# luo-yining/CFDBench

Measured on NVIDIA H100. Metric: fno_rollout_steps_per_sec, higher is better.
Workload: dtype bf16

## Files before the change

### cfdbench_b200/csrc/fno_block_fused.cu

```cuda
#include "fno_common.cuh"
#include "tc_common.cuh"
#include "tc_tma.cuh"
#include <math.h>
#include <string.h>

namespace fno {

constexpr int kFzRows = 16;
constexpr int kFzChunks = kH / kFzRows;
constexpr int kFzWgRows = kFzRows / 2;
constexpr int kFzThreads = 9 * 32;
constexpr int kFzProdWarp = 8;
constexpr int kZK = 2 * kM2;
constexpr int kImgK = 2 * kKX;
constexpr size_t kYmImgBytes = 147456;
constexpr uint32_t kFzStage = 4 * 6144;
constexpr int kFzFFloats = 2 * (2 * kFzRows) * kImgK;
constexpr int kFzEFloats = 2 * kW * kZK;
constexpr uint32_t kFzZtFloats = kC * kZK;
constexpr uint32_t kLboF = (2 * kFzRows / 8) * 128;
constexpr uint32_t kLboO = (kC / 8) * 128;
constexpr uint32_t kFzBoxW = kW, kFzBoxH = 1, kFzBoxC = kC;
constexpr uint32_t kFzRowBytes = kFzBoxW * kFzBoxH * kFzBoxC * 2;
constexpr int kFzXSlots = 4;
constexpr uint32_t kFzW0Bytes = kC * kC * 2;

__host__ __device__ constexpr int fz_x_slot(int n) { return n % kFzXSlots; }
__host__ __device__ constexpr uint32_t fz_x_parity(int n) { return static_cast<uint32_t>(n / kFzXSlots) & 1u; }

struct FzSmem {
  alignas(1024) unsigned char x[2][kFzXSlots][kFzRowBytes];
  alignas(1024) unsigned char st[2][2][kFzRowBytes];
  alignas(128) unsigned char y[2][kFzStage];
  alignas(128) float zt[kFzRows][2][kFzZtFloats];
  alignas(128) float f_hi[kFzFFloats / 2];
  alignas(128) float f_lo[kFzFFloats / 2];
  alignas(128) unsigned char w0[3][kFzW0Bytes];
  alignas(16) float bias[kC];
  alignas(8) uint64_t y_full[2], y_free[2];
  alignas(8) uint64_t x_full[2][kFzXSlots];
};
static_assert(sizeof(FzSmem) <= 232448, "block_fused_kernel: shared memory over the per-block opt-in limit");

__device__ __forceinline__ uint32_t sw128_bf16_offset(int line, int e) {
  return static_cast<uint32_t>(line * 128 + ((((e >> 3) ^ line) & 7) << 4) + (e & 7) * 2);
}

__global__ void __launch_bounds__(kFzThreads, 1)
    block_fused_kernel(const __grid_constant__ CUtensorMap x_map, const __grid_constant__ CUtensorMap out_map,
                       const unsigned char* __restrict__ img, const float* __restrict__ w0t,
                       const float* __restrict__ bias, const float* __restrict__ etab, const float* __restrict__ ftab,
                       int batch) {
  extern __shared__ __align__(1024) unsigned char smem_raw[];
  FzSmem& sm = *reinterpret_cast<FzSmem*>(smem_raw);
  if ((smem_u32(smem_raw) & 1023u) != 0) __trap();
  const int tid = threadIdx.x, lane = tid & 31, warp = tc::warp_index_uniform();
  const int chunk = blockIdx.x % kFzChunks, b0 = blockIdx.x / kFzChunks, bstride = gridDim.x / kFzChunks;
  const int n_units = b0 < batch ? (batch - b0 + bstride - 1) / bstride : 0;

  if (tid == 0) {
    for (int i = 0; i < 2; ++i) {
      mbar_init(&sm.y_full[i], 1);
      mbar_init(&sm.y_free[i], 4);
      for (int s = 0; s < kFzXSlots; ++s) mbar_init(&sm.x_full[i][s], 1);
    }
    fence_mbar_init();
  }
  for (int e = tid; e < kFzFFloats / 2; e += kFzThreads) {
    sm.f_hi[e] = __ldg(ftab + chunk * kFzFFloats + e);
    sm.f_lo[e] = __ldg(ftab + chunk * kFzFFloats + kFzFFloats / 2 + e);
  }
  for (int e = tid; e < kC * kC; e += kFzThreads) {
    const int i = e / kC, o = e % kC;
    const float w = w0t[e];
    const __nv_bfloat16 t1 = __float2bfloat16_rn(w);
    const float r1 = w - __bfloat162float(t1);
    const __nv_bfloat16 t2 = __float2bfloat16_rn(r1);
    const __nv_bfloat16 t3 = __float2bfloat16_rn(r1 - __bfloat162float(t2));
    const uint32_t off = static_cast<uint32_t>(((i >> 3) * (kC / 8) + (o >> 3)) * 128 + (o & 7) * 16 + (i & 7) * 2);
    *reinterpret_cast<__nv_bfloat16*>(sm.w0[0] + off) = t1;
    *reinterpret_cast<__nv_bfloat16*>(sm.w0[1] + off) = t2;
    *reinterpret_cast<__nv_bfloat16*>(sm.w0[2] + off) = t3;
  }
  if (tid < kC) sm.bias[tid] = bias != nullptr ? bias[tid] : 0.f;
  tc::fence_proxy_async_smem();
  __syncthreads();
  pdl_wait();
  pdl_launch_dependents();

  if (warp == kFzProdWarp) {
    if (lane < 2) {
      const int s = lane;
      for (int u = 0; u < n_units; ++u) {
        const unsigned char* src = img + static_cast<size_t>(b0 + u * bstride) * kYmImgBytes;
        for (int pi = 0; pi < 3; ++pi) {
          const int p = s + 2 * pi, f = 3 * u + pi;
          if (f >= 1) mbar_wait(&sm.y_free[s], (f - 1) & 1);
          mbar_expect_tx(&sm.y_full[s], kFzStage);
          bulk_g2s(sm.y[s], src + p * (kFzStage / 2), kFzStage / 2, &sm.y_full[s]);
          bulk_g2s(sm.y[s] + kFzStage / 2, src + kYmImgBytes / 2 + p * (kFzStage / 2), kFzStage / 2, &sm.y_full[s]);
        }
      }
    }
    return;
  }

  const int g = warp >> 2, wq = warp & 3, q = lane & 3, t = tid & 127;
  const int m0 = 16 * wq + (lane >> 2);
  const int n_fills = kFzWgRows * n_units;
  auto x_fill = [&](int n) {
    const int u = n / kFzWgRows, r = n % kFzWgRows, s = fz_x_slot(n);
    mbar_expect_tx(&sm.x_full[g][s], kFzRowBytes);
    tma_load_3d(sm.x[g][s], &x_map, 0, kFzRows * chunk + g + 2 * r, (b0 + u * bstride) * kC, &sm.x_full[g][s]);
  };
  if (t == 0)
    for (int n = 0; n < kFzXSlots && n < n_fills; ++n) x_fill(n);
  const uint32_t w0_s = tc::smem_addr(sm.w0[0]);
  uint32_t e_frag[2][kZK / 8][4];
#pragma unroll
  for (int hl = 0; hl < 2; ++hl)
#pragma unroll
    for (int ks = 0; ks < kZK / 8; ++ks)
#pragma unroll
      for (int j = 0; j < 4; ++j) {
        const uint32_t off = tc::kmajor_offset(m0 + 8 * (j & 1), 8 * ks + q + 4 * (j >> 1), kW) / 4;
        e_frag[hl][ks][j] = __float_as_uint(__ldg(etab + hl * (kFzEFloats / 2) + off));
      }

  for (int u = 0; u < n_units; ++u) {
    const int b = b0 + u * bstride;
    for (int pi = 0; pi < 3; ++pi) {
      const int p = g + 2 * pi, f = 3 * u + pi;
      mbar_wait(&sm.y_full[g], f & 1);
      uint32_t a_hi[6][4], a_lo[6][4];
#pragma unroll
      for (int ks = 0; ks < kImgK / 8; ++ks)
#pragma unroll
        for (int r = 0; r < 4; ++r) {
          const int m = m0 + 8 * (r & 1), kk = 8 * ks + q + 4 * (r >> 1), o = m & 31;
          const uint32_t off = (m >> 5) * 6144 + kk * 128 + (((o >> 3) ^ (kk & 3)) << 5) + (o & 7) * 4;
          a_hi[ks][r] = *reinterpret_cast<const uint32_t*>(sm.y[g] + off);
          a_lo[ks][r] = *reinterpret_cast<const uint32_t*>(sm.y[g] + kFzStage / 2 + off);
        }
      float acc[16];
      tc::wg_fence();
#pragma unroll
      for (int pass = 0; pass < 3; ++pass) {
        const uint32_t fb = tc::smem_addr(pass == 2 ? sm.f_lo : sm.f_hi);
#pragma unroll
        for (int ks = 0; ks < kImgK / 8; ++ks)
          tc::wg_tf32_rs_n32(acc, pass == 1 ? a_lo[ks] : a_hi[ks], tc::make_smem_desc(fb + ks * 2 * kLboF, kLboF, 128),
                             (pass | ks) ? 1u : 0u);
      }
      tc::wg_commit();
      __syncwarp();
      if (lane == 0) mbar_arrive(&sm.y_free[g]);
      tc::wg_wait<0>();
      tc::wg_fence_acc(acc);
      if (pi == 0) tc::named_barrier(1, 256);
#pragma unroll
      for (int hh = 0; hh < 2; ++hh) {
        const int m = m0 + 8 * hh, ky = 2 * p + (m >> 5), o = m & 31;
#pragma unroll
        for (int i = 0; i < 4; ++i)
#pragma unroll
          for (int e = 0; e < 2; ++e) {
            float v = acc[4 * i + 2 * hh + e];
            if (ky == 0 && e == 1) v = sm.bias[o];
            float hi, lo;
            tc::split_tf32(v, hi, lo);
            const uint32_t off = tc::kmajor_offset(o, 2 * ky + e, kC) / 4;
            sm.zt[4 * i + q][0][off] = hi;
            sm.zt[4 * i + q][1][off] = lo;
          }
      }
    }
    tc::fence_proxy_async_smem();
    tc::named_barrier(1, 256);

    float acc[2][16];
    uint32_t x_frag[2][kC / 16][4];
#pragma unroll
    for (int r = 0; r <= kFzWgRows; ++r) {
      if (r < kFzWgRows) {
        const int n = kFzWgRows * u + r, hl = g + 2 * r;
        mbar_wait(&sm.x_full[g][fz_x_slot(n)], fz_x_parity(n));
        const uint32_t a_x = tc::smem_addr(sm.x[g][fz_x_slot(n)]);
#pragma unroll
        for (int ks = 0; ks < kC / 16; ++ks)
          tc::ldmatrix_x4_trans(x_frag[r & 1][ks], a_x + sw128_bf16_offset(16 * ks + 8 * (lane >> 4) + (lane & 7),
                                                                             16 * wq + 8 * ((lane >> 3) & 1)));
        tc::wg_fence();
        const uint32_t b_z[3] = {tc::smem_addr(sm.zt[hl][0]), tc::smem_addr(sm.zt[hl][0]), tc::smem_addr(sm.zt[hl][1])};
#pragma unroll
        for (int pass = 0; pass < 3; ++pass)
#pragma unroll
          for (int ks = 0; ks < kZK / 8; ++ks)
            tc::wg_tf32_rs_n32(acc[r & 1], e_frag[pass == 1][ks],
                               tc::make_smem_desc(b_z[pass] + ks * 2 * kLboO, kLboO, 128), (pass | ks) ? 1u : 0u);
        tc::wg_fence();
#pragma unroll
        for (int term = 0; term < 3; ++term)
#pragma unroll
          for (int ks = 0; ks < kC / 16; ++ks)
            tc::wg_bf16_rs_n32(acc[r & 1], x_frag[r & 1][ks],
                               tc::make_smem_desc(w0_s + term * kFzW0Bytes + ks * 2 * kLboO, kLboO, 128), 1u);
        tc::wg_commit();
      }
      if (r == 0) continue;
      const int rr = r - 1, h = kFzRows * chunk + g + 2 * rr;
      float* d = acc[rr & 1];
      if (r < kFzWgRows) {
        tc::wg_wait<1>();
      } else {
        tc::wg_wait<0>();
      }
      tc::wg_fence_acc(acc[rr & 1]);
      unsigned char* stile = sm.st[g][rr & 1];
#pragma unroll
      for (int i2 = 0; i2 < 2; ++i2) {
        uint32_t v[4];
#pragma unroll
        for (int j = 0; j < 4; ++j) {
          const int i = 2 * i2 + (j >> 1), hh = j & 1;
          const float2 y = gelu_erf2(make_float2(d[4 * i + 2 * hh], d[4 * i + 2 * hh + 1]));
          const __nv_bfloat162 p = __floats2bfloat162_rn(y.x, y.y);
          v[j] = *reinterpret_cast<const uint32_t*>(&p);
        }
        tc::stmatrix_x4_trans(tc::smem_addr(stile) + sw128_bf16_offset(16 * i2 + 8 * (lane >> 4) + (lane & 7),
                                                                       16 * wq + 8 * ((lane >> 3) & 1)),
                              v);
      }
      tc::fence_proxy_async_smem();
      if (t == 0) bulk_wait_group_read<0>();
      tc::named_barrier(2 + g, 128);
      if (t == 0) {
        tma_store_3d(&out_map, stile, 0, h, b * kC);
        bulk_commit_group();
        const int nf = kFzWgRows * u + rr + kFzXSlots;
        if (nf < n_fills) x_fill(nf);
      }
    }
  }
  if (t == 0) bulk_wait_group<0>();
}

void c2r_operand_table(float* host, double s0, double s1);

static float fz_round_tf32_host(double v) {
  float f = static_cast<float>(v);
  uint32_t u;
  memcpy(&u, &f, 4);
  u = (u + 0x1000u) & 0xffffe000u;
  memcpy(&f, &u, 4);
  return f;
}

struct FzTables {
  float* etab = nullptr;
  float* ftab = nullptr;
  int n_sm = 0;
  bool configured = false;
};
static FzTables g_fz[64];

static cudaError_t fz_ensure(int dev, cudaStream_t stream) {
  FzTables& t = g_fz[dev];
  if (t.configured) return cudaSuccess;
  const double two_pi = 6.283185307179586476925286766559;
  static float h_e[kFzEFloats];
  static float h_f[kFzChunks * kFzFFloats];
  c2r_operand_table(h_e, 1.0 / kHW, 2.0 / kHW);
  for (int c = 0; c < kFzChunks; ++c)
    for (int n = 0; n < 2 * kFzRows; ++n) {
      const int h = kFzRows * c + (n >> 1), ri = n & 1;
      for (int k = 0; k < kImgK; ++k) {
        const int rip = k & 1, kxi = 2 * ((k % 24) >> 1) + k / 24, kx = kxi < kM1 ? kxi : kxi + (kH - kKX);
        const double ang = two_pi * ((kx * h) % 64) / 64.0;
        const double val = (ri == rip) ? cos(ang) : (ri == 0 ? -sin(ang) : sin(ang));
        const float hi = fz_round_tf32_host(val);
        const uint32_t off = tc::kmajor_offset(n, k, 2 * kFzRows) / 4;
        h_f[c * kFzFFloats + off] = hi;
        h_f[c * kFzFFloats + kFzFFloats / 2 + off] = fz_round_tf32_host(val - static_cast<double>(hi));
      }
    }
  cudaError_t e = cudaMalloc(&t.etab, sizeof(h_e));
  if (e != cudaSuccess) return e;
  e = cudaMalloc(&t.ftab, sizeof(h_f));
  if (e != cudaSuccess) return e;
  e = cudaMemcpyAsync(t.etab, h_e, sizeof(h_e), cudaMemcpyHostToDevice, stream);
  if (e != cudaSuccess) return e;
  e = cudaMemcpyAsync(t.ftab, h_f, sizeof(h_f), cudaMemcpyHostToDevice, stream);
  if (e != cudaSuccess) return e;
  e = cudaStreamSynchronize(stream);
  if (e != cudaSuccess) return e;
  e = cudaFuncSetAttribute(block_fused_kernel, cudaFuncAttributeMaxDynamicSharedMemorySize, (int)sizeof(FzSmem));
  if (e != cudaSuccess) return e;
  e = cudaDeviceGetAttribute(&t.n_sm, cudaDevAttrMultiProcessorCount, dev);
  if (e != cudaSuccess) return e;
  t.configured = true;
  return cudaSuccess;
}

void block_fused_release(int dev) {
  if (dev < 0 || dev >= 64) return;
  FzTables& t = g_fz[dev];
  if (t.etab) cudaFree(t.etab);
  if (t.ftab) cudaFree(t.ftab);
  t = FzTables();
}

cudaError_t launch_block_fused(const void* ym_img, const void* x, const float* w0t, const float* bias, void* out, int batch,
                               cudaStream_t stream) {
  int dev = 0;
  cudaError_t e = cudaGetDevice(&dev);
  if (e != cudaSuccess) return e;
  if (dev < 0 || dev >= 64) return cudaErrorInvalidDevice;
  e = fz_ensure(dev, stream);
  if (e != cudaSuccess) return e;
  if ((reinterpret_cast<uintptr_t>(x) & 15) || (reinterpret_cast<uintptr_t>(ym_img) & 15) ||
      (reinterpret_cast<uintptr_t>(out) & 15))
    return cudaErrorMisalignedAddress;
  CUtensorMap x_map, out_map;
  const uint64_t planes = static_cast<uint64_t>(batch) * kC;
  e = make_tma_map_3d(&x_map, CU_TENSOR_MAP_DATA_TYPE_BFLOAT16, 2, x, kW, kH, planes, kFzBoxW, kFzBoxH, kFzBoxC);
  if (e != cudaSuccess) return e;
  e = make_tma_map_3d(&out_map, CU_TENSOR_MAP_DATA_TYPE_BFLOAT16, 2, out, kW, kH, planes, kFzBoxW, kFzBoxH, kFzBoxC);
  if (e != cudaSuccess) return e;
  const int slots_max = g_fz[dev].n_sm / kFzChunks;
  const int slots = batch < slots_max ? batch : slots_max;
  return launch_chained(block_fused_kernel, dim3(kFzChunks * slots), dim3(kFzThreads), sizeof(FzSmem), stream, x_map,
                        out_map, static_cast<const unsigned char*>(ym_img), w0t, bias,
                        static_cast<const float*>(g_fz[dev].etab), static_cast<const float*>(g_fz[dev].ftab), batch);
}

}
```

Baseline: 1327.

## Drop producer warp, prefetch spectral image into registers during pointwise stage

Removes the dedicated TMA producer warp and has each warpgroup's thread 0 issue its own bulk copies of the spectral image. The image fragments for the next unit are loaded into registers while the pointwise/GEMM row loop of the current unit runs, and the three inverse-x MMA groups are issued back to back with staggered waits so their stores overlap the next MMA. The zt stores now use float4 vectors over a reorganised staging layout. The cost is much higher register pressure from holding three A-fragment sets, plus a single-slot y buffer whose reuse is now ordered by named barriers.

```diff
diff --git a/cfdbench_b200/csrc/fno_block_fused.cu b/cfdbench_b200/csrc/fno_block_fused.cu
--- a/cfdbench_b200/csrc/fno_block_fused.cu
+++ b/cfdbench_b200/csrc/fno_block_fused.cu
@@ -9,12 +9,12 @@
 constexpr int kFzRows = 16;
 constexpr int kFzChunks = kH / kFzRows;
 constexpr int kFzWgRows = kFzRows / 2;
-constexpr int kFzThreads = 9 * 32;
-constexpr int kFzProdWarp = 8;
+constexpr int kFzThreads = 8 * 32;
 constexpr int kZK = 2 * kM2;
 constexpr int kImgK = 2 * kKX;
 constexpr size_t kYmImgBytes = 147456;
-constexpr uint32_t kFzStage = 4 * 6144;
+constexpr uint32_t kImgKyBytes = kImgK * kC * 4;
+constexpr uint32_t kFzStage = 4 * kImgKyBytes;
 constexpr int kFzFFloats = 2 * (2 * kFzRows) * kImgK;
 constexpr int kFzEFloats = 2 * kW * kZK;
 constexpr uint32_t kFzZtFloats = kC * kZK;
@@ -37,7 +37,7 @@
   alignas(128) float f_lo[kFzFFloats / 2];
   alignas(128) unsigned char w0[3][kFzW0Bytes];
   alignas(16) float bias[kC];
-  alignas(8) uint64_t y_full[2], y_free[2];
+  alignas(8) uint64_t y_full[2];
   alignas(8) uint64_t x_full[2][kFzXSlots];
 };
 static_assert(sizeof(FzSmem) <= 232448, "block_fused_kernel: shared memory over the per-block opt-in limit");
@@ -61,7 +61,6 @@
   if (tid == 0) {
     for (int i = 0; i < 2; ++i) {
       mbar_init(&sm.y_full[i], 1);
-      mbar_init(&sm.y_free[i], 4);
       for (int s = 0; s < kFzXSlots; ++s) mbar_init(&sm.x_full[i][s], 1);
     }
     fence_mbar_init();
@@ -88,23 +87,6 @@
   pdl_wait();
   pdl_launch_dependents();
 
-  if (warp == kFzProdWarp) {
-    if (lane < 2) {
-      const int s = lane;
-      for (int u = 0; u < n_units; ++u) {
-        const unsigned char* src = img + static_cast<size_t>(b0 + u * bstride) * kYmImgBytes;
-        for (int pi = 0; pi < 3; ++pi) {
-          const int p = s + 2 * pi, f = 3 * u + pi;
-          if (f >= 1) mbar_wait(&sm.y_free[s], (f - 1) & 1);
-          mbar_expect_tx(&sm.y_full[s], kFzStage);
-          bulk_g2s(sm.y[s], src + p * (kFzStage / 2), kFzStage / 2, &sm.y_full[s]);
-          bulk_g2s(sm.y[s] + kFzStage / 2, src + kYmImgBytes / 2 + p * (kFzStage / 2), kFzStage / 2, &sm.y_full[s]);
-        }
-      }
-    }
-    return;
-  }
-
   const int g = warp >> 2, wq = warp & 3, q = lane & 3, t = tid & 127;
   const int m0 = 16 * wq + (lane >> 2);
   const int n_fills = kFzWgRows * n_units;
@@ -113,8 +95,18 @@
     mbar_expect_tx(&sm.x_full[g][s], kFzRowBytes);
     tma_load_3d(sm.x[g][s], &x_map, 0, kFzRows * chunk + g + 2 * r, (b0 + u * bstride) * kC, &sm.x_full[g][s]);
   };
-  if (t == 0)
+  const int n_yfills = 3 * n_units;
+  auto y_fill = [&](int f) {
+    const unsigned char* src = img + static_cast<size_t>(b0 + (f / 3) * bstride) * kYmImgBytes +
+                               (g + 2 * (f % 3)) * (kFzStage / 2);
+    mbar_expect_tx(&sm.y_full[g], kFzStage);
+    bulk_g2s(sm.y[g], src, kFzStage / 2, &sm.y_full[g]);
+    bulk_g2s(sm.y[g] + kFzStage / 2, src + kYmImgBytes / 2, kFzStage / 2, &sm.y_full[g]);
+  };
+  if (t == 0) {
+    if (n_yfills > 0) y_fill(0);
     for (int n = 0; n < kFzXSlots && n < n_fills; ++n) x_fill(n);
+  }
   const uint32_t w0_s = tc::smem_addr(sm.w0[0]);
   uint32_t e_frag[2][kZK / 8][4];
 #pragma unroll
@@ -127,54 +119,75 @@
         e_frag[hl][ks][j] = __float_as_uint(__ldg(etab + hl * (kFzEFloats / 2) + off));
       }
 
+  const int o1 = 8 * wq + (lane >> 2);
+  auto load_pair = [&](uint32_t (&a)[2][kImgK / 8][4], int f) {
+    mbar_wait(&sm.y_full[g], f & 1);
+#pragma unroll
+    for (int ks = 0; ks < kImgK / 8; ++ks)
+#pragma unroll
+      for (int r = 0; r < 4; ++r) {
+        const int kk = 8 * ks + q + 4 * (r >> 1);
+        const uint32_t off = (r & 1) * kImgKyBytes + kk * 128 + ((wq ^ (kk & 3)) << 5) + (lane >> 2) * 4;
+        a[0][ks][r] = *reinterpret_cast<const uint32_t*>(sm.y[g] + off);
+        a[1][ks][r] = *reinterpret_cast<const uint32_t*>(sm.y[g] + kFzStage / 2 + off);
+      }
+  };
+  auto issue_pair = [&](float (&acc)[16], const uint32_t (&a)[2][kImgK / 8][4]) {
+    tc::wg_fence();
+#pragma unroll
+    for (int pass = 0; pass < 3; ++pass) {
+      const uint32_t fb = tc::smem_addr(pass == 2 ? sm.f_lo : sm.f_hi);
+#pragma unroll
+      for (int ks = 0; ks < kImgK / 8; ++ks)
+        tc::wg_tf32_rs_n32(acc, a[pass == 1][ks], tc::make_smem_desc(fb + ks * 2 * kLboF, kLboF, 128),
+                           (pass | ks) ? 1u : 0u);
+    }
+    tc::wg_commit();
+  };
+  auto store_pair = [&](const float (&acc)[16], int p) {
+#pragma unroll
+    for (int i = 0; i < 4; ++i) {
+      float v[4] = {acc[4 * i], acc[4 * i + 1], acc[4 * i + 2], acc[4 * i + 3]};
+      if (p == 0) v[1] = sm.bias[o1];
+      float4 hi, lo;
+      tc::split_tf32(v[0], hi.x, lo.x);
+      tc::split_tf32(v[1], hi.y, lo.y);
+      tc::split_tf32(v[2], hi.z, lo.z);
+      tc::split_tf32(v[3], hi.w, lo.w);
+      const uint32_t off = tc::kmajor_offset(o1, 4 * p, kC) / 4;
+      *reinterpret_cast<float4*>(&sm.zt[4 * i + q][0][off]) = hi;
+      *reinterpret_cast<float4*>(&sm.zt[4 * i + q][1][off]) = lo;
+    }
+  };
+  uint32_t a0[2][kImgK / 8][4], a1[2][kImgK / 8][4], a2[2][kImgK / 8][4];
+  auto first_pair = [&](uint32_t (&a)[2][kImgK / 8][4], int f) {
+    load_pair(a, f);
+    tc::named_barrier(2 + g, 128);
+    if (t == 0 && f + 1 < n_yfills) y_fill(f + 1);
+  };
+  if (n_units > 0) {
+    first_pair(a0, 0);
+    first_pair(a1, 1);
+    first_pair(a2, 2);
+  }
+
   for (int u = 0; u < n_units; ++u) {
     const int b = b0 + u * bstride;
-    for (int pi = 0; pi < 3; ++pi) {
-      const int p = g + 2 * pi, f = 3 * u + pi;
-      mbar_wait(&sm.y_full[g], f & 1);
-      uint32_t a_hi[6][4], a_lo[6][4];
-#pragma unroll
-      for (int ks = 0; ks < kImgK / 8; ++ks)
-#pragma unroll
-        for (int r = 0; r < 4; ++r) {
-          const int m = m0 + 8 * (r & 1), kk = 8 * ks + q + 4 * (r >> 1), o = m & 31;
-          const uint32_t off = (m >> 5) * 6144 + kk * 128 + (((o >> 3) ^ (kk & 3)) << 5) + (o & 7) * 4;
-          a_hi[ks][r] = *reinterpret_cast<const uint32_t*>(sm.y[g] + off);
-          a_lo[ks][r] = *reinterpret_cast<const uint32_t*>(sm.y[g] + kFzStage / 2 + off);
-        }
-      float acc[16];
-      tc::wg_fence();
-#pragma unroll
-      for (int pass = 0; pass < 3; ++pass) {
-        const uint32_t fb = tc::smem_addr(pass == 2 ? sm.f_lo : sm.f_hi);
-#pragma unroll
-        for (int ks = 0; ks < kImgK / 8; ++ks)
-          tc::wg_tf32_rs_n32(acc, pass == 1 ? a_lo[ks] : a_hi[ks], tc::make_smem_desc(fb + ks * 2 * kLboF, kLboF, 128),
-                             (pass | ks) ? 1u : 0u);
-      }
-      tc::wg_commit();
-      __syncwarp();
-      if (lane == 0) mbar_arrive(&sm.y_free[g]);
-      tc::wg_wait<0>();
-      tc::wg_fence_acc(acc);
-      if (pi == 0) tc::named_barrier(1, 256);
-#pragma unroll
-      for (int hh = 0; hh < 2; ++hh) {
-        const int m = m0 + 8 * hh, ky = 2 * p + (m >> 5), o = m & 31;
-#pragma unroll
-        for (int i = 0; i < 4; ++i)
-#pragma unroll
-          for (int e = 0; e < 2; ++e) {
-            float v = acc[4 * i + 2 * hh + e];
-            if (ky == 0 && e == 1) v = sm.bias[o];
-            float hi, lo;
-            tc::split_tf32(v, hi, lo);
-            const uint32_t off = tc::kmajor_offset(o, 2 * ky + e, kC) / 4;
-            sm.zt[4 * i + q][0][off] = hi;
-            sm.zt[4 * i + q][1][off] = lo;
-          }
-      }
-    }
+    const bool more = u + 1 < n_units;
+    float acc1[2][16];
+    issue_pair(acc1[0], a0);
+    issue_pair(acc1[1], a1);
+    tc::wg_wait<1>();
+    tc::wg_fence_acc(acc1[0]);
+    tc::named_barrier(1, 256);
+    store_pair(acc1[0], g);
+    issue_pair(acc1[0], a2);
+    tc::wg_wait<1>();
+    tc::wg_fence_acc(acc1[1]);
+    store_pair(acc1[1], g + 2);
+    tc::wg_wait<0>();
+    tc::wg_fence_acc(acc1[0]);
+    store_pair(acc1[0], g + 4);
     tc::fence_proxy_async_smem();
     tc::named_barrier(1, 256);
 
@@ -206,6 +219,9 @@
             tc::wg_bf16_rs_n32(acc[r & 1], x_frag[r & 1][ks],
                                tc::make_smem_desc(w0_s + term * kFzW0Bytes + ks * 2 * kLboO, kLboO, 128), 1u);
         tc::wg_commit();
+        if (more && r == 1) load_pair(a0, 3 * u + 3);
+        if (more && r == 3) load_pair(a1, 3 * u + 4);
+        if (more && r == 5) load_pair(a2, 3 * u + 5);
       }
       if (r == 0) continue;
       const int rr = r - 1, h = kFzRows * chunk + g + 2 * rr;
@@ -239,6 +255,7 @@
         bulk_commit_group();
         const int nf = kFzWgRows * u + rr + kFzXSlots;
         if (nf < n_fills) x_fill(nf);
+        if (more && (r == 1 || r == 3 || r == 5) && 3 * u + 4 + (r >> 1) < n_yfills) y_fill(3 * u + 4 + (r >> 1));
       }
     }
   }
```

Result: faster. 1369 (median of 6 runs) (+3.1%).
